# ruuda/claxon

Measured on AMD Instinct MI355X. Metric: decoded Msamples/s (whole node), 4096-sample stereo 16-bit frames, higher is better.
Workload: dtype i32 (i64 LPC accumulate)

## Files before the change

claxon_amd/csrc/clx_api.hip:

```cpp
#include "clx_kernels.hip"
#include "clx_lanes.hip"
#include "clx_lean.hip"
#include "clx_md5.hip"
#include "clx_index.hip"
#include "clx_window.hip"
#include "clx_mix.hip"
#include "clx_mel.hip"
#include "clx_norm.hip"
#include "clx_add.hip"
#include "clx_reverb.hip"
#include "clx_reverb_fft.hip"
#include "clx_specaug.hip"
#include "clx_splice.hip"

#include <algorithm>
#include <cstdio>
#include <cstdlib>
#include <cstring>
#include <new>
#include <string>
#include <memory>
#include <vector>
#include <unordered_map>
#include <thread>
// ... 501 lines not shown
    for (int i = 0; i < clx_batch::kDepth; ++i) {
        clx_batch::Flight& F = b->flight[i];
        if (F.stream) { (void)hipStreamSynchronize(F.stream); (void)hipStreamDestroy(F.stream); }
        if (F.ev_in) (void)hipEventDestroy(F.ev_in);
        if (F.ev_done) (void)hipEventDestroy(F.ev_done);
        if (F.ev_rice) (void)hipEventDestroy(F.ev_rice);
        if (F.ev_side) (void)hipEventDestroy(F.ev_side);
        if (i != 0 && F.d_sfd) (void)hipFree(F.d_sfd);
        if (i != 0 && F.d_results) (void)hipFree(F.d_results);
        if (i != 0 && F.d_sf_start) (void)hipFree(F.d_sf_start);
        if (i != 0 && F.d_errkey) (void)hipFree(F.d_errkey);
        if (i != 0 && F.d_endbits) (void)hipFree(F.d_endbits);
        if (i != 0 && F.d_taken) (void)hipFree(F.d_taken);
        if (i != 0 && F.d_crc_part) (void)hipFree(F.d_crc_part);
        if (i != 0 && F.d_crc_todo) (void)hipFree(F.d_crc_todo);
        if (i != 0 && F.d_fkey) { (void)hipFree(F.d_slot_frame); (void)hipFree(F.d_first_slot); (void)hipFree(F.d_fkey); }
    }
    if (b->d_stage[clx_batch::kMaxStreams]) (void)hipFree(b->d_stage[clx_batch::kMaxStreams]);
    if (b->ev_up) { (void)hipEventSynchronize(b->ev_up); (void)hipEventDestroy(b->ev_up); }
    if (b->h_up) (void)hipHostFree(b->h_up);
    delete b;
}

namespace {
template <typename T> bool grow(clx_ctx* ctx, T** p, size_t* cap, size_t need, const char* what) {
    if (*p && *cap >= need) return true;
    if (*p) { (void)hipFree(*p); *p = nullptr; *cap = 0; }
    const size_t want = need + need / 4;
    if (!hip_ok(ctx, hipMalloc((void**)p, want ? want : 16), what)) return false;
    *cap = want;
    return true;
}
size_t taken_bytes(uint64_t n_slots) { return (size_t)(2u * ((n_slots + 63) / 64) + 2u) * sizeof(uint32_t); }
int plan_lanes_data(clx_batch* b) {
    clx_ctx* ctx = b->ctx;
    if (b->lanes_planned) return CLX_OK;
    const size_t n = b->n, ns = b->n_slots ? (size_t)b->n_slots : 1, nf = n ? n : 1;
    std::vector<uint32_t> slot_frame(ns), multi(nf), first_slot(nf, 0u);
    b->n_multi = clx_plan_lanes(b->h_frames.data(), n, b->n_slots, slot_frame.data(), multi.data());
    for (size_t i = 0; i < n; ++i) first_slot[i] = b->h_frames[i].first_slot;
    std::vector<clx_window> windows(nf);
    const int cmode = (b->flags & (CLX_NO_COMPOSE | CLX_LANES_GENERAL | CLX_LANES_SPLIT)) ? -1 : (b->flags & CLX_COMPOSE) ? 1 : 0;
    b->n_windows = clx_plan_windows(b->h_frames.data(), n, cmode, windows.data());
    b->any_bps_le16 = b->any_bps_gt16 = false;
    for (size_t i = 0; i < n; ++i) { if (b->h_frames[i].bps <= 16u) b->any_bps_le16 = true; else b->any_bps_gt16 = true; }
    b->general_grid = clx_plan_general_grid(b->h_frames.data(), slot_frame.data(), b->n_slots, b->flags, &b->general_sure);
    {
        uint32_t bs_max = 1;
        for (size_t i = 0; i < n; ++i) bs_max = std::max<uint32_t>(bs_max, b->h_frames[i].block_size);
        b->stage_stride = (bs_max + 3u) & ~3u;
        const uint64_t groups = (b->n_slots + 63) / 64;
        b->stage_groups = (unsigned)std::min<uint64_t>(std::max<uint64_t>(groups, 1), 2 * b->general_sure + 16);
    }
    if (!b->d_most_left && !hip_ok(ctx, hipMalloc((void**)&b->d_most_left, sizeof(uint32_t)), "hipMalloc most_left")) return CLX_API_ERROR;
    if (!b->h_most_left && !hip_ok(ctx, hipHostMalloc((void**)&b->h_most_left, sizeof(uint32_t), hipHostMallocDefault), "hipHostMalloc most_left")) return CLX_API_ERROR;
    *b->h_most_left = 0u;
    if (hipHostGetDevicePointer((void**)&b->h_most_left_dev, b->h_most_left, 0) != hipSuccess) { (void)hipGetLastError(); b->h_most_left_dev = nullptr; }
    if (!hip_ok(ctx, hipMemset(b->d_most_left, 0, sizeof(uint32_t)), "memset most_left")) return CLX_API_ERROR;
    if (!grow(ctx, &b->d_slot_frame, &b->cap[4], ns * sizeof(uint32_t), "hipMalloc slot_frame") ||
        !grow(ctx, &b->d_multi, &b->cap[5], nf * sizeof(uint32_t), "hipMalloc multi") ||
        !grow(ctx, &b->d_sf_start, &b->cap[6], ns * sizeof(uint32_t), "hipMalloc sf_start") ||
        !grow(ctx, &b->d_errkey, &b->cap[7], nf * sizeof(uint32_t), "hipMalloc errkey") ||
        !grow(ctx, &b->d_endbits, &b->cap[8], nf * sizeof(uint64_t), "hipMalloc endbits") ||
        !grow(ctx, &b->d_taken, &b->cap[9], taken_bytes(ns), "hipMalloc taken") ||
        !grow(ctx, &b->d_crc_part, &b->cap[10], ns * sizeof(clx_crc_part), "hipMalloc crc_part") ||
        !grow(ctx, &b->d_crc_todo, &b->cap[11], nf * sizeof(uint32_t), "hipMalloc crc_todo") ||
        !hip_ok(ctx, hipMemset(b->d_taken, 0, taken_bytes(ns)), "memset taken") ||
        !hip_ok(ctx, hipMemset(b->d_crc_part, 0, ns * sizeof(clx_crc_part)), "memset crc_part") ||
        !hip_ok(ctx, hipMemset(b->d_sf_start, 0xff, ns * sizeof(uint32_t)), "memset sf_start") ||
        !hip_ok(ctx, hipMemset(b->d_errkey, 0xff, nf * sizeof(uint32_t)), "memset errkey") ||
        !hip_ok(ctx, hipMemcpy(b->d_slot_frame, slot_frame.data(), ns * sizeof(uint32_t), hipMemcpyHostToDevice), "H2D slot_frame") ||
        !hip_ok(ctx, hipMemcpy(b->d_multi, multi.data(), nf * sizeof(uint32_t), hipMemcpyHostToDevice), "H2D multi")) return CLX_API_ERROR;
    if (!grow(ctx, &b->d_first_slot, &b->cap[12], nf * sizeof(uint32_t), "hipMalloc first_slot") ||
        !hip_ok(ctx, hipMemcpy(b->d_first_slot, first_slot.data(), nf * sizeof(uint32_t), hipMemcpyHostToDevice), "H2D first_slot")) return CLX_API_ERROR;
    if (b->n_windows) {
        if (!grow(ctx, &b->d_windows, &b->cap[13], b->n_windows * sizeof(clx_window), "hipMalloc windows") ||
            !grow(ctx, &b->d_slot_frame_run, &b->cap[14], ns * sizeof(uint32_t), "hipMalloc slot_frame (run)") ||
            !grow(ctx, &b->d_first_slot_run, &b->cap[15], nf * sizeof(uint32_t), "hipMalloc first_slot (run)") ||
            !grow(ctx, &b->d_fkey, &b->cap[16], nf * sizeof(uint32_t), "hipMalloc fkey") ||
            !hip_ok(ctx, hipMemcpy(b->d_windows, windows.data(), b->n_windows * sizeof(clx_window), hipMemcpyHostToDevice), "H2D windows") ||
            !hip_ok(ctx, hipMemcpy(b->d_slot_frame_run, slot_frame.data(), ns * sizeof(uint32_t), hipMemcpyHostToDevice), "H2D slot_frame (run)") ||
            !hip_ok(ctx, hipMemcpy(b->d_first_slot_run, first_slot.data(), nf * sizeof(uint32_t), hipMemcpyHostToDevice), "H2D first_slot (run)") ||
            !hip_ok(ctx, hipMemset(b->d_fkey, 0, nf * sizeof(uint32_t)), "memset fkey")) return CLX_API_ERROR;
    }
    if (!hip_ok(ctx, hipStreamSynchronize(nullptr), "hipStreamSynchronize")) return CLX_API_ERROR;
    b->lanes_planned = true;
    return CLX_OK;
}
int batch_plan_(clx_batch* b, const clx_frame_desc* frames, size_t n, const uint64_t* out_sample_offsets, uint32_t flags);
int launch_pending(clx_batch* b, bool inputs_ready);
int batch_plan(clx_batch* b, const clx_frame_desc* frames, size_t n, const uint64_t* out_sample_offsets, uint32_t flags) {
    const int st = batch_plan_(b, frames, n, out_sample_offsets, flags);
    if (st != CLX_OK) { b->n = 0; b->n_slots = 0; b->n_multi = 0; b->planned_arena_len = (size_t)-1; }
    if (!b->merge_tuned) {
        const uint64_t groups = (b->n_slots + 63) / 64;
        const uint64_t m = groups ? 24576ull / groups : (uint64_t)clx_batch::kMerge;
        b->merge = (int)std::min<uint64_t>(std::max<uint64_t>(m, 1), (uint64_t)clx_batch::kMerge);
    }
    return st;
}
int batch_plan_(clx_batch* b, const clx_frame_desc* frames, size_t n, const uint64_t* out_sample_offsets, uint32_t flags) {
    clx_ctx* ctx = b->ctx;
    if (!b->pend.empty()) {
        if (launch_pending(b) != CLX_OK) { b->launch_failed = false; return CLX_API_ERROR; }
        for (int k = 0; k < clx_batch::kMaxStreams; ++k)
            if (b->mstream[k] && !hip_ok(ctx, hipStreamSynchronize(b->mstream[k]), "hipStreamSynchronize")) return CLX_API_ERROR;
    }
    b->launch_failed = false;
    if (flags & (CLX_OUT_PCM16 | CLX_OUT_PCM24)) {
        const uint32_t wide = (flags & CLX_OUT_PCM24) ? 24u : 16u;
        if ((flags & CLX_OUT_PCM16) && (flags & CLX_OUT_PCM24)) { ctx->last_error = "CLX_OUT_PCM16 and CLX_OUT_PCM24 exclude each other"; return CLX_API_ERROR; }
// ... 98 lines not shown

extern "C" uint64_t clx_batch_slots(const clx_batch* b) { return b ? b->n_slots : 0; }

extern "C" int clx_batch_set_profiling(clx_batch* b, int enable) {
    if (!b) return CLX_API_ERROR;
    b->profiling = enable == 1;
    b->profile_merged = enable == 2;
    b->ev_valid = false;
    return CLX_OK;
}

namespace {
unsigned crc_grid(size_t n) { return (unsigned)std::min<size_t>((n + 3) / 4, 2048); }
unsigned crc_grid_runs(size_t n) { return (unsigned)std::min<size_t>((n + 3) / 4, 256); }
int upload_plan(clx_batch* b, size_t arena_len, hipStream_t stream) {
    clx_ctx* ctx = b->ctx;
    if (b->planned_arena_len == arena_len) return CLX_OK;
    if (b->up_cap < b->n) {
        if (b->up_in_flight) { HIP_TRY(ctx, hipEventSynchronize(b->ev_up)); b->up_in_flight = false; }
        if (b->h_up) (void)hipHostFree(b->h_up);
        b->h_up = nullptr; b->up_cap = 0;
        HIP_TRY(ctx, hipHostMalloc((void**)&b->h_up, (b->n + b->n / 4 + 1) * sizeof(clx_dev_frame), hipHostMallocDefault));
        b->up_cap = b->n + b->n / 4 + 1;
    }
    if (b->up_in_flight) { HIP_TRY(ctx, hipEventSynchronize(b->ev_up)); b->up_in_flight = false; }
    std::memcpy(b->h_up, b->h_frames.data(), b->n * sizeof(clx_dev_frame));
    clx_plan_limits(b->h_descs.data(), b->n, arena_len, b->h_up);
    HIP_TRY(ctx, hipMemcpyAsync(b->d_frames, b->h_up, b->n * sizeof(clx_dev_frame), hipMemcpyHostToDevice, stream));
    if (!b->ev_up) HIP_TRY(ctx, hipEventCreateWithFlags(&b->ev_up, hipEventDisableTiming));
    HIP_TRY(ctx, hipEventRecord(b->ev_up, stream));
    b->up_in_flight = true;
    b->planned_arena_len = arena_len;
    return CLX_OK;
}
int use_lanes(clx_batch* b, size_t arena_len) {
    if (!b->lanes) return 0;
    if ((uint64_t)arena_len + 32ull >= (1ull << 32)) {
        if (b->flags & CLX_PATH_LANES) { b->ctx->last_error = "CLX_PATH_LANES needs arena_len < 4 GiB"; return -1; }
        return 0;
    }
    return 1;
}
unsigned pool_waves(clx_batch* b) {
    if (b->pool_waves) return b->pool_waves;
    int cus = 0;
    if (hipDeviceGetAttribute(&cus, hipDeviceAttributeMultiprocessorCount, b->device) != hipSuccess || cus < 1) cus = 256;
    (void)hipGetLastError();
    b->pool_waves = 12u * (unsigned)cus;
    return b->pool_waves;
}
unsigned device_cus(clx_batch* b) { return pool_waves(b) / 12u; }
template <typename Mark>
bool launch_lanes(clx_batch* b, const clx_runs& runs, unsigned n_runs, bool split, hipStream_t stream, Mark&& mark, clx_pool_state* pool = nullptr,
                  int stage_slot = clx_batch::kMaxStreams) {
    const unsigned groups = (unsigned)((b->n_slots + 63) / 64);
    const bool composed = runs.r[0].fkey != nullptr && b->n_windows && b->n_multi;
    const bool pooled = pool != nullptr && (b->flags & CLX_POOL) && !(b->flags & (CLX_OUT_PCM24 | CLX_OUT_F32)) && !split && !composed && runs.r[0].taken != nullptr && b->any_bps_le16 && !(b->flags & CLX_LANES_GENERAL);
#ifdef CLX_POOL_SCAN_APART
    if (pooled && b->n_multi) {
        if (!mark("clx_k_scan")) return false;
        hipLaunchKernelGGL(clx_k_scan, dim3((unsigned)((b->n_multi + 63) / 64), n_runs), dim3(64), 0, stream, runs,
                           (const clx_dev_frame*)b->d_frames, (const uint32_t*)b->d_multi, (uint32_t)b->n_multi);
    }
    const uint32_t pool_multi = 0u;
#else
    const uint32_t pool_multi = (uint32_t)b->n_multi;
#endif
    if (pooled) {
        if (!mark("clx_k_pool")) return false;
        if (hipMemsetAsync(pool, 0, sizeof(clx_pool_state), stream) != hipSuccess) return false;
        clx_pool_args A;
        A.runs = runs; A.frames = b->d_frames; A.multi = b->d_multi; A.ps = pool; A.order = nullptr; A.dump_all = b->d_dump;
        A.n_runs = n_runs; A.n_slots = (uint32_t)b->n_slots; A.n_multi = pool_multi; A.pad = 0u;
        const uint64_t tickets = (uint64_t)n_runs * ((uint64_t)groups + (pool_multi + 63u) / 64u);
        hipLaunchKernelGGL(clx_k_pool, dim3((unsigned)std::min<uint64_t>(tickets, pool_waves(b))), dim3(64), 0, stream, A);
    }
    else if (b->n_multi) {
        if (!mark("clx_k_scan")) return false;
        if (b->flags & CLX_LANES_GENERAL)
            hipLaunchKernelGGL(clx_k_scan_general, dim3((unsigned)((b->n_multi + 63) / 64), n_runs), dim3(64), 0, stream, runs,
                               (const clx_dev_frame*)b->d_frames, (const uint32_t*)b->d_multi, (uint32_t)b->n_multi);
        else
            hipLaunchKernelGGL(clx_k_scan, dim3((unsigned)((b->n_multi + 63) / 64), n_runs), dim3(64), 0, stream, runs,
                               (const clx_dev_frame*)b->d_frames, (const uint32_t*)b->d_multi, (uint32_t)b->n_multi);
    }
    if (!split) {
        if (composed) {
            if (!mark("clx_k_compose")) return false;
            hipLaunchKernelGGL(clx_k_compose, dim3((unsigned)b->n_windows, n_runs), dim3(CLX_COMPOSE_THREADS), 0, stream, runs, (const clx_window*)b->d_windows);
        }
        const bool p24 = (b->flags & CLX_OUT_PCM24) != 0;
        const bool f32 = (b->flags & CLX_OUT_F32) != 0;
        if (f32 && runs.r[0].taken != nullptr) {
            if (b->any_bps_le16) {
                if (!mark("clx_k_lean_f32")) return false;
                hipLaunchKernelGGL(clx_k_lean_f32, dim3(groups, n_runs), dim3(64), 0, stream, runs,
                                   (const clx_dev_frame*)b->d_frames, (uint32_t)b->n_slots, b->d_dump);
            }
            if (!mark("clx_k_lean24_f32")) return false;
            hipLaunchKernelGGL(clx_k_lean24_f32, dim3(groups, n_runs), dim3(64), 0, stream, runs,
                               (const clx_dev_frame*)b->d_frames, (uint32_t)b->n_slots, b->d_dump);
        }
        if (runs.r[0].taken != nullptr && b->any_bps_le16 && !pooled && !p24 && !f32) {
            if (!mark("clx_k_lean")) return false;
#ifdef CLX_TUNING
            static const unsigned lean_pad = [] { const char* e = std::getenv("CLX_LEAN_LDS_PAD"); return e ? (unsigned)std::strtoul(e, nullptr, 10) : 0u; }();
#else
            const unsigned lean_pad = 0u;
#endif
            hipLaunchKernelGGL(clx_k_lean, dim3(groups, n_runs), dim3(64), lean_pad, stream, runs,
                               (const clx_dev_frame*)b->d_frames, (uint32_t)b->n_slots, b->d_dump);
        }
        if (runs.r[0].taken != nullptr && (b->any_bps_gt16 || p24) && !f32) {
            if (!mark("clx_k_lean24")) return false;
            hipLaunchKernelGGL(clx_k_lean24, dim3(groups, n_runs), dim3(64), 0, stream, runs,
                               (const clx_dev_frame*)b->d_frames, (uint32_t)b->n_slots, b->d_dump);
        }
        unsigned ggrid = groups;
        const bool listed = runs.r[0].taken != nullptr;
        if (listed) {
            if (!mark("clx_k_left")) return false;
            hipLaunchKernelGGL(clx_k_left, dim3((groups + 255) / 256, n_runs), dim3(256), 0, stream, runs, (uint32_t)groups, b->d_most_left, b->h_most_left_dev);
            if (n_runs > 1 && b->general_grid) {
                const unsigned seen = b->h_most_left ? *(volatile uint32_t*)b->h_most_left : 0u;
                ggrid = std::min(groups, std::max(b->general_grid, 2u * seen + 16u));
            }
        }
        clx_runs gruns = runs;
        if (b->flags & (CLX_OUT_PCM16 | CLX_OUT_PCM24 | CLX_OUT_F32)) {
            ggrid = std::min(ggrid, std::max(b->stage_groups, 1u));
            if (b->stage_stride > 4608u) {
                constexpr size_t kStageBudget = size_t(512) << 20;
                const size_t group_bytes = (size_t)64u * b->stage_stride * sizeof(int32_t);
                const size_t floor_per_run = (device_cus(b) + n_runs - 1u) / n_runs;
                ggrid = (unsigned)std::min<size_t>(ggrid, std::max<size_t>(floor_per_run, kStageBudget / (group_bytes * n_runs)));
            }
            const size_t per_run = (size_t)ggrid * 64u * b->stage_stride, need = per_run * n_runs * sizeof(int32_t);
            if (b->stage_cap[stage_slot] < need) {
                if (b->d_stage[stage_slot]) { (void)hipFree(b->d_stage[stage_slot]); b->d_stage[stage_slot] = nullptr; b->stage_cap[stage_slot] = 0; }
                if (!hip_ok(b->ctx, hipMalloc((void**)&b->d_stage[stage_slot], need), "hipMalloc staging rows (narrow output)")) return false;
                b->stage_cap[stage_slot] = need;
            }
            for (unsigned r = 0; r < n_runs; ++r) {
                gruns.r[r].planar = b->d_stage[stage_slot] + per_run * r;
                gruns.r[r].flags |= CLX_RUN_STAGE_BITS(b->stage_stride);
            }
        }
        if (!mark("clx_k_lanes")) return false;
        hipLaunchKernelGGL(clx_k_lanes, dim3(ggrid, n_runs), dim3(64), 0, stream, gruns,
                           (const clx_dev_frame*)b->d_frames, (uint32_t)b->n_slots, b->d_dump);
        hipLaunchKernelGGL(clx_k_lanes_hi, dim3(ggrid, n_runs), dim3(64), 0, stream, gruns,
                           (const clx_dev_frame*)b->d_frames, (uint32_t)b->n_slots, b->d_dump);
    }
    else {
        if (n_runs != 1) return false;
        const clx_run& R = runs.r[0];
        if (!mark("clx_k_lanes2")) return false;
        hipLaunchKernelGGL(clx_k_lanes2, dim3((unsigned)((b->n_slots + 127) / 128)), dim3(256), 0, stream, R.arena, R.alloc_len,
                           (const clx_dev_frame*)b->d_frames, (const uint32_t*)b->d_slot_frame, (uint32_t)b->n_slots,
                           (const uint32_t*)R.sf_start, R.out, R.errkey, R.end_bits, b->d_dump);
    }
    if (!mark("clx_k_finalize")) return false;
    hipLaunchKernelGGL(clx_k_finalize, dim3((unsigned)((b->n + 255) / 256), n_runs), dim3(256), 0, stream, runs,
                       (const clx_dev_frame*)b->d_frames, (uint32_t)b->n, (uint32_t)b->n_slots);
    if (b->flags & CLX_VERIFY_CRC16) {
        if (!mark("clx_k_crc16")) return false;
        hipLaunchKernelGGL(clx_k_crc16_runs, dim3(n_runs > 1 ? crc_grid_runs(b->n) : crc_grid(b->n), n_runs), dim3(256), 0, stream, runs,
                           (const clx_dev_frame*)b->d_frames, (uint32_t)b->n);
    }
    return true;
}
clx_run make_run(const clx_batch* b, const clx_batch::Flight& F, const uint8_t* d_arena, size_t arena_len, int32_t* d_out, bool lean) {
    clx_run R;
    R.arena = d_arena; R.alloc_len = (((uint64_t)arena_len + 15ull) & ~15ull) + 16ull;
    R.out = d_out; R.sf_start = F.d_sf_start; R.errkey = F.d_errkey; R.end_bits = F.d_endbits;
    R.taken = (lean && !(b->flags & CLX_LANES_GENERAL)) ? F.d_taken : nullptr;
    R.results = F.d_results; R.gen = F.gen;
    R.crc_part = F.d_crc_part; R.crc_todo = F.d_crc_todo;
    R.planar = nullptr;
    const bool composed = lean && b->n_windows != 0 && F.d_fkey != nullptr;
    R.slot_frame = composed ? F.d_slot_frame : b->d_slot_frame;
    R.first_slot = composed ? F.d_first_slot : b->d_first_slot;
    R.fkey = composed ? F.d_fkey : nullptr;
    R.flags = ((b->flags & CLX_VERIFY_CRC16) ? CLX_RUN_CRC : 0u) | ((b->flags & CLX_OUT_PCM16) ? CLX_RUN_PCM16 : 0u) | ((b->flags & CLX_OUT_PCM24) ? CLX_RUN_PCM24 : 0u) |
              ((b->flags & CLX_OUT_F32) ? CLX_RUN_F32 : 0u);
    return R;
}
void launch_stage1_waves(clx_batch* b, const uint8_t* d_arena, uint64_t alloc_len, int32_t* d_out, clx_sf_desc* d_sfd, clx_frame_result* d_results,
                         hipStream_t stream) {
#ifdef CLX_TUNING
    static const unsigned k1_pad = [] { const char* e = std::getenv("CLX_K1_LDS_PAD"); return e ? (unsigned)std::strtoul(e, nullptr, 10) : 0u; }();
#else
    const unsigned k1_pad = 0u;
#endif
    hipLaunchKernelGGL(clx_k_residual, dim3((unsigned)b->n), dim3(64), k1_pad, stream,
                       d_arena, alloc_len, (const clx_dev_frame*)b->d_frames, (uint32_t)b->n, d_out, d_sfd, d_results);
}
bool k2_latency_build(const clx_batch* b) {
    const unsigned groups = (unsigned)((b->n_slots + 63) / 64);
    return (b->flags & CLX_K2_LATENCY) ? true : (b->flags & CLX_K2_THROUGHPUT) ? false : groups <= CLX_K2_LATENCY_GROUPS;
}
template <typename Mark>
bool launch_waves(clx_batch* b, const uint8_t* d_arena, uint64_t alloc_len, int32_t* d_out, clx_sf_desc* d_sfd, clx_frame_result* d_results,
                  hipStream_t stream, Mark&& mark, bool k2_latency, hipStream_t side = nullptr, hipEvent_t ev_rice = nullptr,
                  hipEvent_t ev_side = nullptr) {
    if (!mark("clx_k_residual")) return false;
    launch_stage1_waves(b, d_arena, alloc_len, d_out, d_sfd, d_results, stream);
    hipStream_t rest = stream;
    if (side != nullptr) {
        if (hipEventRecord(ev_rice, stream) != hipSuccess || hipStreamWaitEvent(side, ev_rice, 0) != hipSuccess) return false;
        rest = side;
    }
    const unsigned groups = (unsigned)((b->n_slots + 63) / 64);
// ... 47 lines not shown
        if (b->tune_prio) {
            int lo_p = 0, hi_p = 0;
            (void)hipDeviceGetStreamPriorityRange(&lo_p, &hi_p);
            const bool high = ((k & 1) == 0) == (b->tune_prio == 1);
            e0 = hipStreamCreateWithPriority(&st, hipStreamNonBlocking, high ? hi_p : lo_p);
        } else e0 = hipStreamCreateWithFlags(&st, hipStreamNonBlocking);
        if (e0 == hipSuccess) e0 = hipMalloc((void**)&pool, sizeof(clx_pool_state));
        if (e0 == hipSuccess) e0 = hipEventCreateWithFlags(&e_in, hipEventDisableTiming);
        for (auto& e : e_done) if (e0 == hipSuccess) e0 = hipEventCreateWithFlags(&e, hipEventDisableTiming);
        if (e0 != hipSuccess) {
            for (auto& e : e_done) if (e) (void)hipEventDestroy(e);
            if (e_in) (void)hipEventDestroy(e_in);
            if (pool) (void)hipFree(pool);
            if (st) (void)hipStreamDestroy(st);
            return fail("creating an internal stream", e0);
        }
        b->mstream[k] = st; b->m_in[k] = e_in; b->d_pool[k] = pool;
        for (int j = 0; j < clx_batch::kEvRing; ++j) b->m_done[k][j] = e_done[j];
    }
    hipStream_t ms = b->mstream[k];
    if (!inputs_ready) {
        LP_TRY(hipEventRecord(b->m_in[k], b->pend_stream));
        LP_TRY(hipStreamWaitEvent(ms, b->m_in[k], 0));
    }
    {
        uint64_t need[clx_batch::kMaxStreams] = {};
        for (const auto& P : b->pend) {
            const clx_batch::LaunchRef fl = b->flight_launch[P.flight];
            if (fl.count && fl.stream != k) need[fl.stream] = std::max(need[fl.stream], fl.count);
            const auto it = b->out_writer.find(P.out);
            if (it != b->out_writer.end() && it->second.stream != k) need[it->second.stream] = std::max(need[it->second.stream], it->second.count);
        }
        for (int j = 0; j < clx_batch::kMaxStreams; ++j) {
            if (!need[j] || !b->m_count[j]) continue;
            const uint64_t c = (need[j] <= b->m_count[j] && b->m_count[j] - need[j] < (uint64_t)clx_batch::kEvRing) ? need[j] : b->m_count[j];
            LP_TRY(hipStreamWaitEvent(ms, b->m_done[j][(c - 1) % clx_batch::kEvRing], 0));
        }
    }
    if (b->up_in_flight) LP_TRY(hipStreamWaitEvent(ms, b->ev_up, 0));
    if (b->out_writer.size() > 4096u) {
        for (int a = 0; a < clx_batch::kMaxStreams; ++a)
            for (int j = 0; j < clx_batch::kMaxStreams; ++j)
                if (a != j && b->mstream[a] && b->m_count[j])
                    LP_TRY(hipStreamWaitEvent(b->mstream[a], b->m_done[j][(b->m_count[j] - 1) % clx_batch::kEvRing], 0));
        b->out_writer.clear();
    }
    clx_runs runs;
    std::memset(&runs, 0, sizeof runs);
    unsigned n_runs = 0;
    went_out = true;
    for (const auto& P : b->pend) {
        clx_batch::Flight& F = b->flight[P.flight];
        if (++F.gen == 0u) {
            LP_TRY(hipMemsetAsync(F.d_taken, 0, (size_t)((b->n_slots + 63) / 64) * sizeof(uint32_t), ms));
            LP_TRY(hipMemsetAsync(F.d_crc_part, 0, (size_t)std::max<uint64_t>(b->n_slots, 1) * sizeof(clx_crc_part), ms));
            F.gen = 1u;
        }
        if (F.scratch_stale) {
            LP_TRY(hipMemsetAsync(F.d_sf_start, 0xff, (size_t)std::max<uint64_t>(b->n_slots, 1) * sizeof(uint32_t), ms));
            LP_TRY(hipMemsetAsync(F.d_errkey, 0xff, std::max<size_t>(b->n, 1) * sizeof(uint32_t), ms));
            LP_TRY(hipMemsetAsync(F.d_taken + (b->n_slots + 63) / 64, 0, sizeof(uint32_t), ms));
            F.scratch_stale = false;
        }
        runs.r[n_runs++] = make_run(b, F, P.arena, P.arena_len, P.out, true);
    }
    int nk = 0;
    auto mark = [&](const char* name) -> bool {
        if (!b->profile_merged) return true;
        if (nk > (name ? clx_batch::kMaxKernels - 1 : clx_batch::kMaxKernels)) { ctx->last_error = "more kernels in one launch than profiling marks"; return false; }
        if (name) b->kname[nk] = name;
        return hip_ok(ctx, hipEventRecord(b->ev[nk++], ms), "hipEventRecord");
    };
    if (!(launch_lanes(b, runs, n_runs, false, ms, mark, b->d_pool[k], k) && hipGetLastError() == hipSuccess)) return fail("kernel launch", hipSuccess);
    if (b->profile_merged) { if (!mark(nullptr)) return fail("hipEventRecord", hipSuccess); b->n_kernels = nk - 1; b->ev_valid = true; b->ev_runs = (int)n_runs; }
    LP_TRY(hipEventRecord(b->m_done[k][b->m_count[k] % clx_batch::kEvRing], ms));
#undef LP_TRY
    ++b->m_count[k];
    for (const auto& P : b->pend) {
        b->out_writer[P.out] = clx_batch::LaunchRef{ k, b->m_count[k] };
        b->flight_launch[P.flight] = clx_batch::LaunchRef{ k, b->m_count[k] };
    }
    b->m_unwaited[k] = true;
    b->pend.clear();
    ++b->n_merged;
    ++b->launches_since_wait;
    return CLX_OK;
}
int wait_flights(clx_batch* b, hipStream_t stream) {
    if (launch_pending(b) != CLX_OK) { b->launch_failed = false; return CLX_API_ERROR; }
    if (b->launch_failed) {
        b->launch_failed = false;
        b->ctx->last_error = "an earlier merged launch of this batch failed; its submissions were dropped";
        return CLX_API_ERROR;
    }
    b->launches_since_wait = 0;
    for (int k = 0; k < clx_batch::kMaxStreams; ++k)
        if (b->m_unwaited[k]) { HIP_TRY(b->ctx, hipStreamWaitEvent(stream, b->m_done[k][(b->m_count[k] - 1) % clx_batch::kEvRing], 0)); b->m_unwaited[k] = false; }
    for (auto& F : b->flight)
        if (F.pending) {
            HIP_TRY(b->ctx, hipStreamWaitEvent(stream, F.ev_done, 0));
            if (F.side_pending) HIP_TRY(b->ctx, hipStreamWaitEvent(stream, F.ev_side, 0));
            F.pending = false; F.side_pending = false;
        }
    return CLX_OK;
}
}

extern "C" int clx_batch_run(clx_batch* b, const uint8_t* d_arena, size_t arena_len, int32_t* d_out, void* stream_) {
    if (!b || !b->ctx) return CLX_API_ERROR;
    clx_ctx* ctx = b->ctx;
    if (b->n == 0) return CLX_OK;
    if (!d_arena || !d_out) { ctx->last_error = "null device pointer"; return CLX_API_ERROR; }
    if (((uintptr_t)d_arena & 15u) != 0) { ctx->last_error = "device arena must be 16-byte aligned"; return CLX_API_ERROR; }
    HIP_TRY(ctx, hipSetDevice(ctx->device));
    hipStream_t stream = stream_ ? (hipStream_t)stream_ : ctx->stream;
    if (wait_flights(b, stream) != CLX_OK) return CLX_API_ERROR;
    b->last_slot = -1;
    b->last_stream = stream;
    if (upload_plan(b, arena_len, stream) != CLX_OK) return CLX_API_ERROR;
    const uint64_t alloc_len = (((uint64_t)arena_len + 15ull) & ~15ull) + 16ull;

    int nk = 0;
    auto mark = [&](const char* name) -> bool {
        if (!b->profiling) return true;
        if (nk > (name ? clx_batch::kMaxKernels - 1 : clx_batch::kMaxKernels)) { ctx->last_error = "more kernels in one run than profiling marks"; return false; }
        if (name) b->kname[nk] = name;
        return hip_ok(ctx, hipEventRecord(b->ev[nk++], stream), "hipEventRecord");
    };
    const int lanes = use_lanes(b, arena_len);
    if (lanes < 0) return CLX_API_ERROR;
    if (lanes) {
        const bool split = (b->flags & CLX_LANES_SPLIT) ? true : (b->flags & CLX_LANES_FUSED) ? false : b->choice.lanes_split;
        clx_batch::Flight& F0 = b->flight[0];
        F0.d_results = b->d_results; F0.d_sf_start = b->d_sf_start; F0.d_errkey = b->d_errkey; F0.d_endbits = b->d_endbits; F0.d_taken = b->d_taken;
        F0.d_crc_part = b->d_crc_part; F0.d_crc_todo = b->d_crc_todo;
        F0.d_slot_frame = b->d_slot_frame_run; F0.d_first_slot = b->d_first_slot_run; F0.d_fkey = b->d_fkey;
        if (++F0.gen == 0u) {
            HIP_TRY(ctx, hipMemsetAsync(b->d_taken, 0, (size_t)((b->n_slots + 63) / 64) * sizeof(uint32_t), stream));
            HIP_TRY(ctx, hipMemsetAsync(b->d_crc_part, 0, (size_t)std::max<uint64_t>(b->n_slots, 1) * sizeof(clx_crc_part), stream));
            F0.gen = 1u;
        }
        if (F0.scratch_stale) {
            HIP_TRY(ctx, hipMemsetAsync(b->d_sf_start, 0xff, (size_t)std::max<uint64_t>(b->n_slots, 1) * sizeof(uint32_t), stream));
            HIP_TRY(ctx, hipMemsetAsync(b->d_errkey, 0xff, std::max<size_t>(b->n, 1) * sizeof(uint32_t), stream));
            HIP_TRY(ctx, hipMemsetAsync(b->d_taken + (b->n_slots + 63) / 64, 0, sizeof(uint32_t), stream));
            F0.scratch_stale = false;
        }
        clx_runs runs;
        std::memset(&runs, 0, sizeof runs);
        runs.r[0] = make_run(b, F0, d_arena, arena_len, d_out, !split);
        if (!launch_lanes(b, runs, 1u, split, stream, mark) || hipGetLastError() != hipSuccess) {
            F0.scratch_stale = true;
            ctx->last_error = "a launch of the lane kernels failed";
            return CLX_API_ERROR;
        }
    } else {
        clx_batch::Flight& F0 = b->flight[0];
        if (F0.sfd_stale) { HIP_TRY(ctx, hipMemsetAsync(b->d_sfd, 0, (size_t)std::max<uint64_t>(b->n_slots, 1) * sizeof(clx_sf_desc), stream)); F0.sfd_stale = false; }
        if (!launch_waves(b, d_arena, alloc_len, d_out, b->d_sfd, b->d_results, stream, mark, k2_latency_build(b))) return CLX_API_ERROR;
    }
    if (b->profiling) { if (!mark(nullptr)) return CLX_API_ERROR; b->n_kernels = nk - 1; b->ev_valid = true; }
    HIP_TRY(ctx, hipGetLastError());
    return CLX_OK;
}

namespace {
bool submit_wants_lanes(const clx_batch* b) {
    return (b->flags & CLX_PATH_LANES) ? true : (b->flags & CLX_PATH_WAVES) ? false : b->lanes_submit;
}
}

extern "C" int clx_batch_submit_lanes(const clx_batch* b) { return b && !b->profiling && submit_wants_lanes(b) && !(b->flags & CLX_LANES_SPLIT) ? 1 : 0; }

extern "C" int clx_batch_submit_depth(const clx_batch* b) {
    if (!b) return 1;
    if (b->profiling) return 1;
    if (submit_wants_lanes(b)) return (b->flags & CLX_LANES_SPLIT) ? 1 : b->merge * b->n_streams;
    return (b->flags & CLX_K2_THROUGHPUT) ? 1 : clx_batch::kDepthWaves;
}

extern "C" int clx_batch_submit_merge(const clx_batch* b) { return (b && clx_batch_submit_lanes(b)) ? b->merge : 1; }

extern "C" int clx_batch_submit(clx_batch* b, const uint8_t* d_arena, size_t arena_len, int32_t* d_out, void* stream_) {
    if (!b || !b->ctx) return CLX_API_ERROR;
    clx_ctx* ctx = b->ctx;
    if (b->n == 0) return CLX_OK;
    if (!d_arena || !d_out) { ctx->last_error = "null device pointer"; return CLX_API_ERROR; }
    if (((uintptr_t)d_arena & 15u) != 0) { ctx->last_error = "device arena must be 16-byte aligned"; return CLX_API_ERROR; }
    bool want_lanes = submit_wants_lanes(b);
    if (want_lanes && (uint64_t)arena_len + 32ull >= (1ull << 32)) {
        if (b->flags & CLX_PATH_LANES) { ctx->last_error = "CLX_PATH_LANES needs arena_len < 4 GiB"; return CLX_API_ERROR; }
// ... 1750 lines not shown
```

claxon_amd/csrc/clx_lanes.hip:

```cpp
#include <hip/hip_runtime.h>
#include <stdint.h>

#include <clx_intrin.h>

#include "../../include/claxon_hip.h"
#include <type_traits>
#include "clx_device.h"

#define CLX_LERR(status, msg) (((uint32_t)(status) << 16) | (uint32_t)(msg))

struct LaneReader {
    const uint8_t* arena;
    uint32_t origin;
    uint32_t pos;
    uint32_t limit;
    uint32_t err;
};

__device__ __forceinline__ uint32_t clx_lpeek32(const LaneReader& r, uint32_t pos) {
    const uint32_t boff = r.origin + ((pos >> 3) & ~3u);
    const uint32_t* p = reinterpret_cast<const uint32_t*>(r.arena + boff);
    const uint64_t w = ((uint64_t)__builtin_bswap32(p[0]) << 32) | __builtin_bswap32(p[1]);
    return (uint32_t)((w << (pos & 31u)) >> 32);
}
// ... 963 lines not shown
    if (!active) { bs = 0; r.err = 1u; }
    Ring g;
    g.src = reinterpret_cast<const uint32_t*>(arena + r.origin);
    g.avail_dw = (uint32_t)((arena_alloc_len > r.origin ? arena_alloc_len - r.origin : 0ull) >> 2);
    g.fill = 0; g.npend = 0; g.pend0 = make_uint4(0u, 0u, 0u, 0u); g.pend1 = g.pend0; g.pend2 = g.pend0; g.fast_lim = 0;

    SfHead h = { 1u, 0u, 0u, 1u };
    if (active && !r.err) h = clx_lparse_sf_header(r, clx_channel_bps(fr, ch));

    const uint32_t decor = active ? fr.channel_assignment : 0u;
    const uint32_t pbs = (uint32_t)__builtin_amdgcn_update_dpp(0, (int)(active ? bs : 0u), 0xB1, 0xF, 0xF, false);
    const uint32_t pd = (uint32_t)__builtin_amdgcn_update_dpp(0, (int)decor, 0xB1, 0xF, 0xF, false);
    const bool pair_ok = active && decor != CLX_CH_INDEPENDENT && pbs == bs && pd == decor;

    uint32_t nmax = active ? bs : 0u;
    uint32_t omax = (active && !r.err && h.kind >= 2u) ? h.order : 0u;
#pragma unroll
    for (int s = 32; s >= 1; s >>= 1) {
        uint32_t a = __shfl_xor(nmax, s, 64); nmax = a > nmax ? a : nmax;
        uint32_t b = __shfl_xor(omax, s, 64); omax = b > omax ? b : omax;
    }
    int32_t* const row = narrow ? out + (size_t)lane * stride : out + (active ? fr.out_off + (uint64_t)ch * fr.block_size : 0ull);
    const bool row_aligned = (((uintptr_t)row) & 15u) == 0u;
    uint32_t end_pos = r.pos, err = r.err;
    int32_t* const dump = dump_all + (size_t)slot * 16u;
    if ((omax > 12u) != HI) return;
    if (nmax != 0u) {
        if (HI)               clx_lanes_run<32>(r, g, L.ring[lane], L.stage[lane], h, bs, decor, pair_ok, row, row_aligned, nmax, omax, lane, &end_pos, &err, out, dump);
        else if (omax <= 4u)  clx_lanes_run<4>(r, g, L.ring[lane], L.stage[lane], h, bs, decor, pair_ok, row, row_aligned, nmax, omax, lane, &end_pos, &err, out, dump);
        else if (omax <= 8u)  clx_lanes_run<8>(r, g, L.ring[lane], L.stage[lane], h, bs, decor, pair_ok, row, row_aligned, nmax, omax, lane, &end_pos, &err, out, dump);
        else                  clx_lanes_run<12>(r, g, L.ring[lane], L.stage[lane], h, bs, decor, pair_ok, row, row_aligned, nmax, omax, lane, &end_pos, &err, out, dump);
    }
    if (narrow) clx_narrow_row(R, fr, ch, active ? bs : 0u, row, narrow);
    if (active) {
        if (err) clx_report_error(errkey, f, ch, err);
        else if (ch + 1u == fr.n_channels) end_bits[f] = (uint64_t)(end_pos - o);
    }
    CLX_TL_END(3, grp);
}
template <bool HI>
__device__ __forceinline__ void clx_lanes_fused(const clx_runs& runs, const clx_dev_frame* __restrict__ frames,
                 uint32_t n_slots, int32_t* __restrict__ dump_all) {
    __shared__ LanesLds L;
    const clx_run& R = runs.r[blockIdx.y];
    if (R.taken == nullptr) { clx_lanes_group<HI>(L, R, frames, n_slots, dump_all, blockIdx.x); return; }
    const uint32_t* const left = R.taken + (n_slots + 63u) / 64u;
    const uint32_t n_left = left[0];
#pragma unroll 1
    for (uint32_t i = blockIdx.x; i < n_left; i += gridDim.x) {
        clx_lanes_group<HI>(L, R, frames, n_slots, dump_all, left[1u + i]);
        clx_wave_sync();
    }
}
extern "C" __global__ __launch_bounds__(256)
void clx_k_left(const clx_runs runs, uint32_t n_groups, uint32_t* __restrict__ most_left, uint32_t* __restrict__ most_left_host) {
    const clx_run& R = runs.r[blockIdx.y];
    const uint32_t g = blockIdx.x * 256u + threadIdx.x;
    if (g >= n_groups || R.taken == nullptr) return;
    if (R.taken[g] != R.gen) {
        uint32_t* const left = R.taken + n_groups;
        const uint32_t i = atomicAdd(&left[0], 1u);
        left[1u + i] = g;
        if (most_left != nullptr && atomicMax(most_left, i + 1u) < i + 1u && most_left_host != nullptr) *(volatile uint32_t*)most_left_host = i + 1u;
    }
}
extern "C" __global__ __launch_bounds__(64)
void clx_k_lanes(const clx_runs runs, const clx_dev_frame* __restrict__ frames, uint32_t n_slots,
                 int32_t* __restrict__ dump_all) {
    clx_lanes_fused<false>(runs, frames, n_slots, dump_all);
}
extern "C" __global__ __launch_bounds__(64)
void clx_k_lanes_hi(const clx_runs runs, const clx_dev_frame* __restrict__ frames, uint32_t n_slots,
                    int32_t* __restrict__ dump_all) {
    clx_lanes_fused<true>(runs, frames, n_slots, dump_all);
}

struct Lanes2Lds {
    uint32_t ring[64][CLX_ROW];
    int4 tile[2][4][64];
    clx_sf_desc desc[64];
};

__device__ __forceinline__ void clx_l2_publish(clx_sf_desc* d, const LaneState<32>& S, const SfHead& h, uint32_t n, bool with_coefs) {
    d->n = (uint16_t)n;
    d->order = (uint8_t)((n != 0u && h.kind >= 2u) ? h.order : 0u);
    d->wasted = (uint8_t)h.wasted;
    d->flags = 0; d->decor = 0; d->out_base = 0;
    if (!with_coefs) {
        d->shift = 0; d->lim_log2 = 23;
#pragma unroll
        for (int j = 0; j < 32; ++j) d->coef[j] = 0;
    } else {
        d->shift = (uint8_t)S.shift;
        d->lim_log2 = (uint8_t)(S.lim < 0 ? 0xffu : (uint32_t)(31 - __clz(S.lim)));
#pragma unroll
        for (int j = 0; j < 32; ++j) d->coef[j] = (int16_t)S.c[j];
    }
}

__device__ __forceinline__ void clx_rice_wave(LaneState<32>& S, Ring& g, uint32_t* ringrow, int4 (*tile)[4][64], clx_sf_desc* desc, const SfHead h,
                                              uint32_t bs, uint32_t n, uint32_t nmax, uint32_t omax, int lane) {
    LaneReader& r = S.r;
    const uint32_t sw = ((uint32_t)lane >> 2) & 3u;
    bool published = false;
    uint32_t i0 = (omax + 4u + 15u) & ~15u;
    if (i0 > nmax) i0 = (nmax + 15u) & ~15u;
    const uint32_t nturn = (nmax + 15u) >> 4;
    bool ring_ready = false;
    for (uint32_t T = 0; T < nturn; ++T) {
        int4* const out4 = &tile[T & 1u][0][0];
        if (ring_ready) {
            const uint32_t tb = 16u * T;
            clx_ring_pump(g, ringrow, r.pos, r.limit);
            const bool live = (n != 0u) && !r.err && tb < n;
            const LeanKind K = clx_lean_kind<32>(S, h);
            const int lean_mode = clx_lean_mode(live, K, S.phase);
// ... 223 lines not shown
#pragma unroll
        for (int j = 0; j < 32; ++j) { S.c[j] = 0; S.hist[j] = 0; }
        const uint32_t n = r.err ? 0u : bs;
        S.phase = 3u; S.cval = 0; S.trans_at = 0xffffffffu; S.transitioned = false;
        S.order = 0; S.shift = 0; S.lim = 0x7fffffff;
        S.k = 0; S.k1 = 1; S.pcnt = 0; S.next_cnt = 0; S.per = 0; S.parts_left = 0; S.rice2 = 0;
        if (n) {
            if (h.kind == 0u) { S.cval = clx_lread_signed(S.r, h.sf_bps); S.phase = 2u; }
            else if (h.kind == 1u) S.phase = 0u;
            else {
                if (bs < h.order) S.r.err = CLX_LERR(CLX_FORMAT_ERROR, h.kind == 2u ? CLX_MSG_FIXED_ORDER_GT_BLOCK : CLX_MSG_LPC_ORDER_GT_BLOCK);
                else { S.phase = 0u; S.trans_at = h.order; }
            }
        }
        clx_l2_publish(&L.desc[lane], S, h, S.r.err ? 0u : n, false);
        clx_wg_barrier();
        clx_rice_wave(S, g, L.ring[lane], L.tile, &L.desc[lane], h, bs, S.r.err ? 0u : n, nmax, omax, lane);
        if (active) {
            if (S.r.err) clx_report_error(errkey, f, ch, S.r.err);
            else if (ch + 1u == fr.n_channels) end_bits[f] = (uint64_t)(S.r.pos - o);
        }
    } else {
        clx_wg_barrier();
        K2Slot S;
        S.d = &L.desc[lane];
        const bool valid = f != 0xffffffffu;
        S.n = valid ? fr.block_size : 0u;
        S.order = valid ? S.d->order : 0u; S.shift = 0; S.wasted = valid ? S.d->wasted : 0u;
        S.decor = valid ? fr.channel_assignment : 0u; S.lim_log2 = 0;
        S.row = out + (valid ? fr.out_off + (uint64_t)ch * fr.block_size : 0ull);
        if (S.n == 0u) { S.order = 0; S.wasted = 0; S.decor = 0; }
        const uint32_t pn = (uint32_t)__builtin_amdgcn_update_dpp(0, (int)S.n, 0xB1, 0xF, 0xF, false);
        const uint32_t pd = (uint32_t)__builtin_amdgcn_update_dpp(0, (int)S.decor, 0xB1, 0xF, 0xF, false);
        S.pair_ok = (S.decor != CLX_CH_INDEPENDENT) && pn == S.n && pd == S.decor && S.n != 0u;
        uint32_t omax = S.order;
#pragma unroll
        for (int s = 32; s >= 1; s >>= 1) { const uint32_t b = __shfl_xor(omax, s, 64); omax = b > omax ? b : omax; }
        int32_t* const dump = dump_all + (size_t)(group * 64u + (uint32_t)lane) * CLX_BLK;
        const bool al = (S.n == 0u) || ((((uintptr_t)S.row) & 15u) == 0u && (S.n & 3u) == 0u);
        if (__all(al)) {
            if (omax <= 4u)       clx_pf_wave_mode<4, true>(L.tile, out, S, dump, nturn, lane);
            else if (omax <= 8u)  clx_pf_wave_mode<8, true>(L.tile, out, S, dump, nturn, lane);
            else if (omax <= 12u) clx_pf_wave_mode<12, true>(L.tile, out, S, dump, nturn, lane);
            else                  clx_pf_wave_mode<32, true>(L.tile, out, S, dump, nturn, lane);
        } else {
            if (omax <= 4u)       clx_pf_wave_mode<4, false>(L.tile, out, S, dump, nturn, lane);
            else if (omax <= 8u)  clx_pf_wave_mode<8, false>(L.tile, out, S, dump, nturn, lane);
            else if (omax <= 12u) clx_pf_wave_mode<12, false>(L.tile, out, S, dump, nturn, lane);
            else                  clx_pf_wave_mode<32, false>(L.tile, out, S, dump, nturn, lane);
        }
    }
}

extern "C" __global__ __launch_bounds__(256)
void clx_k_finalize(const clx_runs runs, const clx_dev_frame* __restrict__ frames, uint32_t n_frames, uint32_t n_slots) {
    const clx_run& R = runs.r[blockIdx.y];
    const uint32_t f = blockIdx.x * 256u + threadIdx.x;
    if (f >= n_frames) return;
    if (f == 0u && R.taken != nullptr) R.taken[(n_slots + 63u) / 64u] = 0u;
    const uint32_t key = R.errkey[f];
    const clx_dev_frame fr = frames[f];
    clx_frame_result r;
    if (key == 0xffffffffu) {
        r.status = CLX_OK; r.msg = CLX_MSG_NONE; r.end_bit = R.end_bits[f];
        if (!(fr.flags & 1u) && ((r.end_bit + 7ull) & ~7ull) + 16ull > (uint64_t)fr.limit_bits) {
            r.status = CLX_IO_ERROR; r.msg = CLX_MSG_UNEXPECTED_EOF;
        }
    }
    else { r.status = (int32_t)((key >> 16) & 0xffu); r.msg = key & 0xffffu; r.end_bit = 0; }
    if (R.flags & CLX_RUN_CRC) {
        uint32_t todo = 0u;
        if (r.status == CLX_OK && !(fr.flags & 1u)) {
            todo = 1u;
            if (((r.end_bit + 7ull) & ~7ull) + 16ull == (uint64_t)fr.limit_bits) {
                bool all = true;
                uint32_t sum = 0u, par = 0u, at = 0u;
                const uint32_t nch = fr.n_channels;
                const uint32_t dend = R.crc_part[fr.first_slot + nch - 1u].db;
                for (uint32_t c = 0; c < nch; ++c) {
                    const clx_crc_part p = R.crc_part[fr.first_slot + c];
                    all = all && p.gen == R.gen && p.da == at && p.db >= p.da && p.db <= dend;
                    if (!all) break;
                    at = p.db;
                    sum ^= clx_crct_shift(p.rx & 0x7fffu, dend - p.db);
                    par ^= p.rx >> 31;
                }
                if (all) {
                    todo = 0u;
                    if (sum != 0u || par != 0u) { r.status = CLX_FORMAT_ERROR; r.msg = CLX_MSG_FRAME_CRC_MISMATCH; }
                }
            }
        }
        R.crc_todo[f] = todo;
    }
    R.results[f] = r;
    R.errkey[f] = 0xffffffffu;
    for (uint32_t c = 1; c < fr.n_channels; ++c) R.sf_start[fr.first_slot + c] = 0xffffffffu;
}
```

Baseline: 665,200.

## Fuse leftover-group listing with finalize and shrink fallback grid when nothing is left

Adds a tail path for multi-run batches: when the host-visible hints show no leftover groups and no pending CRC work from earlier batches, a single clx_k_tail kernel lists leftover groups and finalizes frames whose slot groups are already settled. The general lanes kernel then runs with a tiny grid, and finalize and CRC16 run as small "rest" kernels that exit early unless a tail flag was raised. The aim is to remove separate left, finalize and CRC launches and the oversized fallback grid in the common case. The hints now have two slots updated with a CAS loop, the taken buffer needs room for an extra flag word, and the decision depends on stale host hints from previous batches.

```diff
diff --git a/claxon_amd/csrc/clx_api.hip b/claxon_amd/csrc/clx_api.hip
--- a/claxon_amd/csrc/clx_api.hip
+++ b/claxon_amd/csrc/clx_api.hip
@@ -577,11 +577,11 @@
         const uint64_t groups = (b->n_slots + 63) / 64;
         b->stage_groups = (unsigned)std::min<uint64_t>(std::max<uint64_t>(groups, 1), 2 * b->general_sure + 16);
     }
-    if (!b->d_most_left && !hip_ok(ctx, hipMalloc((void**)&b->d_most_left, sizeof(uint32_t)), "hipMalloc most_left")) return CLX_API_ERROR;
-    if (!b->h_most_left && !hip_ok(ctx, hipHostMalloc((void**)&b->h_most_left, sizeof(uint32_t), hipHostMallocDefault), "hipHostMalloc most_left")) return CLX_API_ERROR;
-    *b->h_most_left = 0u;
+    if (!b->d_most_left && !hip_ok(ctx, hipMalloc((void**)&b->d_most_left, 2 * sizeof(uint32_t)), "hipMalloc most_left")) return CLX_API_ERROR;
+    if (!b->h_most_left && !hip_ok(ctx, hipHostMalloc((void**)&b->h_most_left, 2 * sizeof(uint32_t), hipHostMallocDefault), "hipHostMalloc most_left")) return CLX_API_ERROR;
+    b->h_most_left[0] = b->h_most_left[1] = 0u;
     if (hipHostGetDevicePointer((void**)&b->h_most_left_dev, b->h_most_left, 0) != hipSuccess) { (void)hipGetLastError(); b->h_most_left_dev = nullptr; }
-    if (!hip_ok(ctx, hipMemset(b->d_most_left, 0, sizeof(uint32_t)), "memset most_left")) return CLX_API_ERROR;
+    if (!hip_ok(ctx, hipMemset(b->d_most_left, 0, 2 * sizeof(uint32_t)), "memset most_left")) return CLX_API_ERROR;
     if (!grow(ctx, &b->d_slot_frame, &b->cap[4], ns * sizeof(uint32_t), "hipMalloc slot_frame") ||
         !grow(ctx, &b->d_multi, &b->cap[5], nf * sizeof(uint32_t), "hipMalloc multi") ||
         !grow(ctx, &b->d_sf_start, &b->cap[6], ns * sizeof(uint32_t), "hipMalloc sf_start") ||
@@ -786,8 +786,42 @@
 unsigned device_cus(clx_batch* b) { return pool_waves(b) / 12u; }
 template <typename Mark>
 bool launch_lanes(clx_batch* b, const clx_runs& runs, unsigned n_runs, bool split, hipStream_t stream, Mark&& mark, clx_pool_state* pool = nullptr,
-                  int stage_slot = clx_batch::kMaxStreams) {
+                  int stage_slot = clx_batch::kMaxStreams, std::string* why = nullptr) {
     const unsigned groups = (unsigned)((b->n_slots + 63) / 64);
+    const bool listed = !split && runs.r[0].taken != nullptr;
+    const bool narrow = (b->flags & (CLX_OUT_PCM16 | CLX_OUT_PCM24 | CLX_OUT_F32)) != 0;
+    const unsigned seen = b->h_most_left ? ((volatile uint32_t*)b->h_most_left)[0] : 0u, seen_crc = b->h_most_left ? ((volatile uint32_t*)b->h_most_left)[1] : 0u;
+    unsigned ggrid = groups;
+    if (listed && n_runs > 1 && b->general_grid) ggrid = std::min(groups, std::max(b->general_grid, 2u * seen + 16u));
+    constexpr unsigned kTailGrid = 8u;
+    const bool empty_tail = listed && n_runs > 1 && !narrow && b->general_sure == 0 && seen == 0u && seen_crc == 0u && b->h_most_left_dev != nullptr;
+    if (empty_tail) ggrid = std::min(groups, kTailGrid);
+    clx_runs gruns = runs;
+    if (!split && narrow) {
+        ggrid = std::min(ggrid, std::max(b->stage_groups, 1u));
+        if (b->stage_stride > 4608u) {
+            constexpr size_t kStageBudget = size_t(512) << 20;
+            const size_t group_bytes = (size_t)64u * b->stage_stride * sizeof(int32_t);
+            const size_t floor_per_run = (device_cus(b) + n_runs - 1u) / n_runs;
+            ggrid = (unsigned)std::min<size_t>(ggrid, std::max<size_t>(floor_per_run, kStageBudget / (group_bytes * n_runs)));
+        }
+        const size_t per_run = (size_t)ggrid * 64u * b->stage_stride, need = per_run * n_runs * sizeof(int32_t);
+        if (b->stage_cap[stage_slot] < need) {
+            if (b->d_stage[stage_slot]) { (void)hipFree(b->d_stage[stage_slot]); b->d_stage[stage_slot] = nullptr; b->stage_cap[stage_slot] = 0; }
+            const hipError_t e = hipMalloc((void**)&b->d_stage[stage_slot], need);
+            if (e != hipSuccess) {
+                (void)hipGetLastError();
+                b->ctx->last_error = std::string("hipMalloc staging rows (narrow output): ") + hipGetErrorString(e);
+                if (why) *why = b->ctx->last_error;
+                return false;
+            }
+            b->stage_cap[stage_slot] = need;
+        }
+        for (unsigned r = 0; r < n_runs; ++r) {
+            gruns.r[r].planar = b->d_stage[stage_slot] + per_run * r;
+            gruns.r[r].flags |= CLX_RUN_STAGE_BITS(b->stage_stride);
+        }
+    }
     const bool composed = runs.r[0].fkey != nullptr && b->n_windows && b->n_multi;
     const bool pooled = pool != nullptr && (b->flags & CLX_POOL) && !(b->flags & (CLX_OUT_PCM24 | CLX_OUT_F32)) && !split && !composed && runs.r[0].taken != nullptr && b->any_bps_le16 && !(b->flags & CLX_LANES_GENERAL);
 #ifdef CLX_POOL_SCAN_APART
@@ -850,35 +884,13 @@
             hipLaunchKernelGGL(clx_k_lean24, dim3(groups, n_runs), dim3(64), 0, stream, runs,
                                (const clx_dev_frame*)b->d_frames, (uint32_t)b->n_slots, b->d_dump);
         }
-        unsigned ggrid = groups;
-        const bool listed = runs.r[0].taken != nullptr;
-        if (listed) {
+        if (empty_tail) {
+            if (!mark("clx_k_tail")) return false;
+            hipLaunchKernelGGL(clx_k_tail, dim3((unsigned)((std::max<size_t>(b->n, groups) + 255) / 256), n_runs), dim3(256), 0, stream, runs,
+                               (const clx_dev_frame*)b->d_frames, (uint32_t)b->n, (uint32_t)b->n_slots, b->d_most_left, b->h_most_left_dev);
+        } else if (listed) {
             if (!mark("clx_k_left")) return false;
             hipLaunchKernelGGL(clx_k_left, dim3((groups + 255) / 256, n_runs), dim3(256), 0, stream, runs, (uint32_t)groups, b->d_most_left, b->h_most_left_dev);
-            if (n_runs > 1 && b->general_grid) {
-                const unsigned seen = b->h_most_left ? *(volatile uint32_t*)b->h_most_left : 0u;
-                ggrid = std::min(groups, std::max(b->general_grid, 2u * seen + 16u));
-            }
-        }
-        clx_runs gruns = runs;
-        if (b->flags & (CLX_OUT_PCM16 | CLX_OUT_PCM24 | CLX_OUT_F32)) {
-            ggrid = std::min(ggrid, std::max(b->stage_groups, 1u));
-            if (b->stage_stride > 4608u) {
-                constexpr size_t kStageBudget = size_t(512) << 20;
-                const size_t group_bytes = (size_t)64u * b->stage_stride * sizeof(int32_t);
-                const size_t floor_per_run = (device_cus(b) + n_runs - 1u) / n_runs;
-                ggrid = (unsigned)std::min<size_t>(ggrid, std::max<size_t>(floor_per_run, kStageBudget / (group_bytes * n_runs)));
-            }
-            const size_t per_run = (size_t)ggrid * 64u * b->stage_stride, need = per_run * n_runs * sizeof(int32_t);
-            if (b->stage_cap[stage_slot] < need) {
-                if (b->d_stage[stage_slot]) { (void)hipFree(b->d_stage[stage_slot]); b->d_stage[stage_slot] = nullptr; b->stage_cap[stage_slot] = 0; }
-                if (!hip_ok(b->ctx, hipMalloc((void**)&b->d_stage[stage_slot], need), "hipMalloc staging rows (narrow output)")) return false;
-                b->stage_cap[stage_slot] = need;
-            }
-            for (unsigned r = 0; r < n_runs; ++r) {
-                gruns.r[r].planar = b->d_stage[stage_slot] + per_run * r;
-                gruns.r[r].flags |= CLX_RUN_STAGE_BITS(b->stage_stride);
-            }
         }
         if (!mark("clx_k_lanes")) return false;
         hipLaunchKernelGGL(clx_k_lanes, dim3(ggrid, n_runs), dim3(64), 0, stream, gruns,
@@ -893,6 +905,17 @@
         hipLaunchKernelGGL(clx_k_lanes2, dim3((unsigned)((b->n_slots + 127) / 128)), dim3(256), 0, stream, R.arena, R.alloc_len,
                            (const clx_dev_frame*)b->d_frames, (const uint32_t*)b->d_slot_frame, (uint32_t)b->n_slots,
                            (const uint32_t*)R.sf_start, R.out, R.errkey, R.end_bits, b->d_dump);
+    }
+    if (empty_tail) {
+        if (!mark("clx_k_finalize")) return false;
+        hipLaunchKernelGGL(clx_k_finalize_rest, dim3(std::min((unsigned)((b->n + 255) / 256), kTailGrid), n_runs), dim3(256), 0, stream, runs,
+                           (const clx_dev_frame*)b->d_frames, (uint32_t)b->n, (uint32_t)b->n_slots);
+        if (b->flags & CLX_VERIFY_CRC16) {
+            if (!mark("clx_k_crc16")) return false;
+            hipLaunchKernelGGL(clx_k_crc16_rest, dim3(std::min(crc_grid_runs(b->n), kTailGrid), n_runs), dim3(256), 0, stream, runs,
+                               (const clx_dev_frame*)b->d_frames, (uint32_t)b->n, (uint32_t)b->n_slots);
+        }
+        return true;
     }
     if (!mark("clx_k_finalize")) return false;
     hipLaunchKernelGGL(clx_k_finalize, dim3((unsigned)((b->n + 255) / 256), n_runs), dim3(256), 0, stream, runs,
@@ -1046,7 +1069,7 @@
     for (const auto& P : b->pend) {
         clx_batch::Flight& F = b->flight[P.flight];
         if (++F.gen == 0u) {
-            LP_TRY(hipMemsetAsync(F.d_taken, 0, (size_t)((b->n_slots + 63) / 64) * sizeof(uint32_t), ms));
+            LP_TRY(hipMemsetAsync(F.d_taken, 0, taken_bytes(b->n_slots), ms));
             LP_TRY(hipMemsetAsync(F.d_crc_part, 0, (size_t)std::max<uint64_t>(b->n_slots, 1) * sizeof(clx_crc_part), ms));
             F.gen = 1u;
         }
@@ -1065,7 +1088,8 @@
         if (name) b->kname[nk] = name;
         return hip_ok(ctx, hipEventRecord(b->ev[nk++], ms), "hipEventRecord");
     };
-    if (!(launch_lanes(b, runs, n_runs, false, ms, mark, b->d_pool[k], k) && hipGetLastError() == hipSuccess)) return fail("kernel launch", hipSuccess);
+    std::string why;
+    if (!(launch_lanes(b, runs, n_runs, false, ms, mark, b->d_pool[k], k, &why) && hipGetLastError() == hipSuccess)) return fail(why.empty() ? "kernel launch" : why.c_str(), hipSuccess);
     if (b->profile_merged) { if (!mark(nullptr)) return fail("hipEventRecord", hipSuccess); b->n_kernels = nk - 1; b->ev_valid = true; b->ev_runs = (int)n_runs; }
     LP_TRY(hipEventRecord(b->m_done[k][b->m_count[k] % clx_batch::kEvRing], ms));
 #undef LP_TRY
@@ -1130,7 +1154,7 @@
         F0.d_crc_part = b->d_crc_part; F0.d_crc_todo = b->d_crc_todo;
         F0.d_slot_frame = b->d_slot_frame_run; F0.d_first_slot = b->d_first_slot_run; F0.d_fkey = b->d_fkey;
         if (++F0.gen == 0u) {
-            HIP_TRY(ctx, hipMemsetAsync(b->d_taken, 0, (size_t)((b->n_slots + 63) / 64) * sizeof(uint32_t), stream));
+            HIP_TRY(ctx, hipMemsetAsync(b->d_taken, 0, taken_bytes(b->n_slots), stream));
             HIP_TRY(ctx, hipMemsetAsync(b->d_crc_part, 0, (size_t)std::max<uint64_t>(b->n_slots, 1) * sizeof(clx_crc_part), stream));
             F0.gen = 1u;
         }
diff --git a/claxon_amd/csrc/clx_lanes.hip b/claxon_amd/csrc/clx_lanes.hip
--- a/claxon_amd/csrc/clx_lanes.hip
+++ b/claxon_amd/csrc/clx_lanes.hip
@@ -1039,6 +1039,11 @@
         clx_wave_sync();
     }
 }
+__device__ __forceinline__ void clx_hint_raise(uint32_t* dev, uint32_t* host, uint32_t v) {
+    if (dev == nullptr || atomicMax(dev, v) >= v || host == nullptr) return;
+    uint32_t cur = __atomic_load_n(host, __ATOMIC_RELAXED);
+    while (cur < v && !__atomic_compare_exchange_n(host, &cur, v, true, __ATOMIC_RELAXED, __ATOMIC_RELAXED)) { }
+}
 extern "C" __global__ __launch_bounds__(256)
 void clx_k_left(const clx_runs runs, uint32_t n_groups, uint32_t* __restrict__ most_left, uint32_t* __restrict__ most_left_host) {
     const clx_run& R = runs.r[blockIdx.y];
@@ -1048,7 +1053,7 @@
         uint32_t* const left = R.taken + n_groups;
         const uint32_t i = atomicAdd(&left[0], 1u);
         left[1u + i] = g;
-        if (most_left != nullptr && atomicMax(most_left, i + 1u) < i + 1u && most_left_host != nullptr) *(volatile uint32_t*)most_left_host = i + 1u;
+        clx_hint_raise(most_left, most_left_host, i + 1u);
     }
 }
 extern "C" __global__ __launch_bounds__(64)
@@ -1378,12 +1383,8 @@
     }
 }
 
-extern "C" __global__ __launch_bounds__(256)
-void clx_k_finalize(const clx_runs runs, const clx_dev_frame* __restrict__ frames, uint32_t n_frames, uint32_t n_slots) {
-    const clx_run& R = runs.r[blockIdx.y];
-    const uint32_t f = blockIdx.x * 256u + threadIdx.x;
-    if (f >= n_frames) return;
-    if (f == 0u && R.taken != nullptr) R.taken[(n_slots + 63u) / 64u] = 0u;
+__device__ __forceinline__ bool clx_finalize_frame(const clx_run& R, const clx_dev_frame* __restrict__ frames, uint32_t f) {
+    bool crc_left = false;
     const uint32_t key = R.errkey[f];
     const clx_dev_frame fr = frames[f];
     clx_frame_result r;
@@ -1418,8 +1419,61 @@
             }
         }
         R.crc_todo[f] = todo;
+        crc_left = todo != 0u;
     }
     R.results[f] = r;
     R.errkey[f] = 0xffffffffu;
     for (uint32_t c = 1; c < fr.n_channels; ++c) R.sf_start[fr.first_slot + c] = 0xffffffffu;
-}
+    return crc_left;
+}
+extern "C" __global__ __launch_bounds__(256)
+void clx_k_finalize(const clx_runs runs, const clx_dev_frame* __restrict__ frames, uint32_t n_frames, uint32_t n_slots) {
+    const clx_run& R = runs.r[blockIdx.y];
+    const uint32_t f = blockIdx.x * 256u + threadIdx.x;
+    if (f >= n_frames) return;
+    if (f == 0u && R.taken != nullptr) R.taken[(n_slots + 63u) / 64u] = 0u;
+    (void)clx_finalize_frame(R, frames, f);
+}
+
+__device__ __forceinline__ uint32_t* clx_tail_flag(const clx_run& R, uint32_t n_slots) { return R.taken + 2u * ((n_slots + 63u) / 64u) + 1u; }
+__device__ __forceinline__ bool clx_tail_settled(const clx_run& R, const clx_dev_frame* __restrict__ frames, uint32_t f) {
+    const uint32_t s0 = R.first_slot[f], s1 = s0 + frames[f].n_channels - 1u;
+    return R.taken[s0 >> 6] == R.gen && R.taken[s1 >> 6] == R.gen;
+}
+extern "C" __global__ __launch_bounds__(256)
+void clx_k_tail(const clx_runs runs, const clx_dev_frame* __restrict__ frames, uint32_t n_frames, uint32_t n_slots,
+                uint32_t* __restrict__ hints, uint32_t* __restrict__ hints_host) {
+    const clx_run& R = runs.r[blockIdx.y];
+    const uint32_t t = blockIdx.x * 256u + threadIdx.x;
+    const uint32_t n_groups = (n_slots + 63u) / 64u;
+    bool raise = false;
+    if (t < n_groups && R.taken[t] != R.gen) {
+        uint32_t* const left = R.taken + n_groups;
+        const uint32_t i = atomicAdd(&left[0], 1u);
+        left[1u + i] = t;
+        clx_hint_raise(hints, hints_host, i + 1u);
+        raise = true;
+    }
+    if (t < n_frames) {
+        if (!clx_tail_settled(R, frames, t)) raise = true;
+        else if (clx_finalize_frame(R, frames, t)) {
+            clx_hint_raise(hints != nullptr ? hints + 1 : nullptr, hints_host != nullptr ? hints_host + 1 : nullptr, 1u);
+            raise = true;
+        }
+    }
+    if (raise) *clx_tail_flag(R, n_slots) = R.gen;
+}
+extern "C" __global__ __launch_bounds__(256)
+void clx_k_finalize_rest(const clx_runs runs, const clx_dev_frame* __restrict__ frames, uint32_t n_frames, uint32_t n_slots) {
+    const clx_run& R = runs.r[blockIdx.y];
+    if (*clx_tail_flag(R, n_slots) != R.gen) return;
+    if (blockIdx.x == 0u && threadIdx.x == 0u) R.taken[(n_slots + 63u) / 64u] = 0u;
+    for (uint32_t f = blockIdx.x * 256u + threadIdx.x; f < n_frames; f += gridDim.x * 256u)
+        if (!clx_tail_settled(R, frames, f)) (void)clx_finalize_frame(R, frames, f);
+}
+extern "C" __global__ __launch_bounds__(256)
+void clx_k_crc16_rest(const clx_runs runs, const clx_dev_frame* __restrict__ frames, uint32_t n_frames, uint32_t n_slots) {
+    const clx_run& R = runs.r[blockIdx.y];
+    if (*clx_tail_flag(R, n_slots) != R.gen) return;
+    clx_crc16_frames(R.arena, frames, n_frames, R.results, R.crc_todo);
+}
```

Result: slower. 656,000 (-1.4%).
